# agordon/fastx_toolkit

Measured on AMD Instinct MI355X. Metric: Mreads/s (150 bp) quality-trim+filter, higher is better.
Workload: dtype u8

## Files before the change

fastx_toolkit_amd/csrc/fxg_device.h:

```cpp
#pragma once
#include <hip/hip_runtime.h>
#include <stdint.h>
#include <cstdio>
#include <cstring>

#include "../../include/fxg.h"

typedef unsigned int       u32;
typedef unsigned long long u64;
typedef unsigned int u32x4 __attribute__((ext_vector_type(4)));

#define FXG_HD __host__ __device__ __forceinline__
#define FXG_PLAN_FAIL(...) do { snprintf(err, cap, __VA_ARGS__); return FXG_E_INVALID; } while (0)
static inline int fxg_text_check_len(unsigned long long text_len, char *err, size_t cap) { if (text_len > 0xFFFFFFF0ull) FXG_PLAN_FAIL("text block too large (%llu bytes)", text_len); return FXG_OK; }
static inline bool fxg_text_lpr_ok(int lpr) { return lpr == 4 || lpr == 2; }

#if defined(FXG_ABLATION) || defined(FXG_DBG_BITS)
#define FXG_DBG(a, bit) ((a).debug & (bit))
#else
#define FXG_DBG(a, bit) 0u
#endif

#define FXG_BLOCK 256
#define FXG_WAVES (FXG_BLOCK / 64)
// ... 64 lines not shown
    u32  nf_keep_n;
    u32  rev_dw;
    u64 *extra;
    const uint8_t  *clip_src;
    u64  clip_total;
    u32  clip_stride;
    const uint16_t *wlen;
    float *clip_ck;
    u32  clip_ck_rows;
    u32  clip_ptab_rows;
    u32  clip_ptab_stride;
    u32  clip_ptab_cols;
    u32  clip_ptab_dia1;
    char adapter[100];
    uint8_t clip_ptab_row[256];
};

__device__ __forceinline__ u32 fxg_lane() { return threadIdx.x & 63u; }

FXG_HD u32 fxg_ge_flags(u32 w, u32 K) { return (((w & 0x7f7f7f7fu) + K) | w) & 0x80808080u; }

FXG_HD u32 fxg_pack4(u32 f)
{
    u32 t = f >> 7;
    t |= t >> 7;
    t |= t >> 14;
    return t & 0xFu;
}

FXG_HD u32 fxg_mask16(u32x4 v, u32 K)
// ... 549 lines not shown
```

fastx_toolkit_amd/csrc/fxg_engine.hip:

```cpp
#include "fxg_host.h"
#include "fxg_text.h"
#include "fxg_history.h"
#include "fxg_stats.h"
#include "fxg_fallback.h"
#include "fxg_barcode.h"
#include "fxg_reflow.h"

extern "C" int fxg_abi_version(void) { return FXG_ABI_VERSION; }

extern "C" int fxg_ctx_create(int device_id, fxg_ctx **out)
{
    if (!out) return FXG_E_INVALID;
    *out = nullptr;
    int ndev = 0;
    if (hipGetDeviceCount(&ndev) != hipSuccess || ndev <= 0 || device_id < 0 || device_id >= ndev) return FXG_E_HIP;
    fxg_ctx *c = (fxg_ctx *)calloc(1, sizeof(fxg_ctx));
    if (!c) return FXG_E_NOMEM;
    c->device = device_id;
    hipDeviceProp_t prop;
    if (hipSetDevice(device_id) != hipSuccess || hipGetDeviceProperties(&prop, device_id) != hipSuccess ||
        hipStreamCreateWithFlags(&c->own_stream, hipStreamNonBlocking) != hipSuccess) { fxg_ctx_destroy(c); return FXG_E_HIP; }
    c->cus = prop.multiProcessorCount;
    c->stream = c->own_stream;
    { const char *e = getenv("FXG_BLOCKS_PER_CU"); c->env_blocks_per_cu = (e && atoi(e) > 0 && atoi(e) <= 16) ? atoi(e) : 0; }
    { const char *e = getenv("FXG_WORKERS"); c->env_workers = (e && atoi(e) > 0) ? atoi(e) : 0; }
    { const char *e = getenv("FXG_NSCAN"); c->env_nscan = (e && atoi(e) > 0 && atoi(e) <= 64) ? atoi(e) : 0; }
    { const char *e = getenv("FXG_TEST_SCAN_TIMEOUT"); c->test_force_timeout = (e && atoi(e) > 0) ? 1 : 0; }
    { const char *e = getenv("FXG_TICKET_GROUPS"); c->env_ticket_groups = (e && atoi(e) > 0 && atoi(e) <= FXG_TICKET_GROUPS) ? atoi(e) : 0; }
    if (hipEventCreate(&c->ev0) != hipSuccess || hipEventCreate(&c->ev1) != hipSuccess ||
        hipMalloc((void **)&c->errflag, (FXG_CTRL_WORDS + FXG_TICKET_GROUPS * FXG_TICKET_STRIDE) * sizeof(u32)) != hipSuccess ||
        hipMalloc((void **)&c->counters_scratch, FXG_NCOUNTERS * sizeof(u64)) != hipSuccess) { fxg_ctx_destroy(c); return FXG_E_HIP; }
    *out = c;
    return FXG_OK;
}

extern "C" void fxg_ctx_destroy(fxg_ctx *c)
{
    if (!c) return;
    (void)hipSetDevice(c->device);
    if (c->stream) (void)hipStreamSynchronize(c->stream);
    (void)hipFree(c->status); (void)hipFree(c->errflag); (void)hipFree(c->counters_scratch);
// ... 152 lines not shown
    return fxg_launch_plan(c, pl, (u64 *)out->counters);
}

static int fxg_launch_clip(fxg_ctx *c, FxgPlan &pl, u64 *ctr)
{
    int rc;
#define FXG_CLIP_TRY_UNIT(K) if ((rc = FXG_CLIP_UNIT_FN(K)(c, pl, ctr)) != FXG_CLIP_NOT_MINE) return rc;
    FXG_CLIP_FOR_UNITS(FXG_CLIP_TRY_UNIT)
#undef FXG_CLIP_TRY_UNIT
    return fxg_fail(c, FXG_E_INVALID, "no clip instance %d", pl.amax);
}

static int fxg_launch_plan(fxg_ctx *c, FxgPlan &pl, u64 *ctr)
{
    if (pl.rows_nw) {
        if (pl.rows_h == 2) {
            if (pl.rows_nw == 26) return fxg_launch_tiles(c, fxg_kernel_rows<26, 2>, "fxg_kernel_rows<26,2> qtrim+qfilter", pl.ka, pl.lds, ctr, 64u, true);
            return fxg_launch_tiles(c, fxg_kernel_rows<38, 2>, "fxg_kernel_rows<38,2> qtrim+qfilter", pl.ka, pl.lds, ctr, 64u, true);
        }
        switch (pl.rows_nw) {
        case 10: return fxg_launch_tiles(c, fxg_kernel_rows_multi<10, 4>, "fxg_kernel_rows_multi<10,4> qtrim+qfilter", pl.ka, pl.lds, ctr, 64u, true);
        case 14: return fxg_launch_tiles(c, fxg_kernel_rows_multi<14, 3>, "fxg_kernel_rows_multi<14,3> qtrim+qfilter", pl.ka, pl.lds, ctr, 64u, true);
        case 20: return fxg_launch_tiles(c, fxg_kernel_rows_multi<20, 2>, "fxg_kernel_rows_multi<20,2> qtrim+qfilter", pl.ka, pl.lds, ctr, 64u, true);
        case 26: return fxg_launch_tiles(c, fxg_kernel_rows<26>, "fxg_kernel_rows<26> qtrim+qfilter", pl.ka, pl.lds, ctr, 64u, true);
        default: return fxg_launch_tiles(c, fxg_kernel_rows<38>, "fxg_kernel_rows<38> qtrim+qfilter", pl.ka, pl.lds, ctr, 64u, true);
        }
    }
    if (pl.group_a) {
        if (pl.amax == 0) return fxg_launch_tiles(c, fxg_kernel_tiles<0, 0>, "fxg_kernel_tiles<0,0> qtrim+qfilter", pl.ka, pl.lds, ctr);
        return fxg_launch_clip(c, pl, ctr);
    }
    if (pl.mask) return fxg_launch_tiles(c, fxg_kernel_tiles<0, 3>, "fxg_kernel_tiles<0,3> mask", pl.ka, pl.lds, ctr);
    if (pl.artifacts) return fxg_launch_tiles(c, fxg_kernel_tiles<0, 4>, "fxg_kernel_tiles<0,4> base census", pl.ka, pl.lds, ctr);
    if (pl.rev && pl.ka.rev_dw) return fxg_launch_tiles(c, fxg_kernel_tiles<0, 5>, "fxg_kernel_tiles<0,5> revcomp[+ftrim], dword-aligned windows", pl.ka, pl.lds, ctr);
    if (pl.rev) return fxg_launch_tiles(c, fxg_kernel_tiles<0, 2>, "fxg_kernel_tiles<0,2> revcomp[+ftrim]", pl.ka, pl.lds, ctr);
    return fxg_launch_tiles(c, fxg_kernel_tiles<0, 1>, "fxg_kernel_tiles<0,1> ftrim", pl.ka, pl.lds, ctr);
}

extern "C" int fxg_run_quality_stats(fxg_ctx *c, const fxg_batch *in, uint64_t *d_hist, uint32_t hist_cols)
{
    if (!c) return FXG_E_INVALID;
// ... 530 lines not shown
```

fastx_toolkit_amd/csrc/fxg_host.h:

```cpp
#pragma once
#include <hip/hip_runtime.h>

#include <dlfcn.h>
#include <fcntl.h>
#include <cerrno>
#include <cstdarg>
#include <cstdio>
#include <cstdlib>
#include <cstring>
#include <unistd.h>

#include "fxg_plan.h"
#include "fxg_rows.h"

struct FxgTextState;

struct fxg_ctx {
    int device;
    int cus;
    hipStream_t own_stream;
    hipStream_t stream;
    hipEvent_t ev0, ev1;
#define FXG_KEV_RING 64
    hipEvent_t kev0[FXG_KEV_RING], kev1[FXG_KEV_RING];
    int profiling;
    u64 kev_count;
    int kev_ready;
    u64 *status;
    size_t status_cap;
    u32 epoch;
    void *attr_kernel[8];
    u32 attr_lds[8];
    int attr_per_cu[8];
    int attr_next;
    void *lds_kernel[32];
    u32 lds_max[32];
    int env_blocks_per_cu, env_ticket_groups;
    int env_workers, env_nscan;
    u32 *errflag;
    u64 *counters_scratch;
    u64 *text_ws;
    size_t text_ws_cap;
    FxgTextState *text_state;
    int hist_on;
    u32 hist_wcap;
    int hist_cur;
    uint8_t *hist_buf[2];
    u32 *hist_w;
    uint8_t *hist_ws;
    size_t hist_ws_cap;
    float *clip_ck;
    size_t clip_ck_cap;
    u32 *stats_ws;
// ... 68 lines not shown
        FXG_HIP(c, hipFuncSetAttribute((const void *)kernel, hipFuncAttributeMaxDynamicSharedMemorySize, (int)lds));
        if (k >= 0) { c->lds_kernel[k] = (void *)kernel; c->lds_max[k] = lds; }
    }
    FXG_HIP(c, hipOccupancyMaxActiveBlocksPerMultiprocessor(per_cu, kernel, (int)block, lds));
    if (*per_cu < 1) return fxg_fail(c, FXG_E_INVALID, "%s does not fit on a CU (lds=%u)", kname, lds);
    int slot = -1;
    for (int i = 0; i < 8; ++i) if (!c->attr_kernel[i]) { slot = i; break; }
    if (slot < 0) { slot = c->attr_next; c->attr_next = (c->attr_next + 1) % 8; }
    c->attr_kernel[slot] = (void *)kernel; c->attr_lds[slot] = lds; c->attr_per_cu[slot] = *per_cu;
    return FXG_OK;
}

#define FXG_STATUS_WORDS(cap) (3 * (size_t)(cap) + 2 * ((size_t)(cap) / 256 + 2))

template <typename K>
static int fxg_launch_tiles(fxg_ctx *c, K kernel, const char *kname, FxgKArgs &ka, u32 lds, u64 *counters, u32 block = FXG_TBLOCK, bool rows_kernel = false, u64 ck_per_wg = 0)
{
    FXG_HIP(c, hipSetDevice(c->device));
    int per_cu = 0;
    FXG_TRY(fxg_kernel_fit(c, kernel, kname, lds, &per_cu, block));
    const int most = block == 64u ? 16 : 8;
    int use = per_cu > most ? most : per_cu;
    if (c->env_blocks_per_cu > 0) use = c->env_blocks_per_cu;
    u64 workers = (u64)c->cus * (u64)use;
    if (c->env_workers > 0 && workers > (u64)c->env_workers) workers = (u64)c->env_workers;
    if (workers > ka.ntiles) workers = ka.ntiles;
    if (workers < 1) workers = 1;
    ka.nscan = !ka.compact ? 0u : (rows_kernel && workers >= 64u * FXG_ROWS_NSCAN ? (u32)FXG_ROWS_NSCAN : 1u);
    if (ka.compact && rows_kernel && c->env_nscan > 0) ka.nscan = (u32)c->env_nscan;
    const u64 grid = workers + ka.nscan;

    if (ka.compact) {
        bool fresh = false;
        const size_t cap = (size_t)ka.ntiles + (size_t)ka.ntiles / 4 + 1024;
        FXG_TRY(fxg_ws_grow(c, c->status, c->status_cap, ka.ntiles, cap, &fresh, FXG_STATUS_WORDS(cap) * sizeof(u64)));
        c->epoch = c->epoch >= 255u ? 1u : c->epoch + 1u;
        if (fresh || c->epoch == 1u) FXG_HIP(c, hipMemsetAsync(c->status, 0, FXG_STATUS_WORDS(c->status_cap) * sizeof(u64), c->stream));
        ka.agg = c->status;
        ka.pfx = c->status + c->status_cap;
        ka.bbase = c->status + 3 * c->status_cap;
        ka.tag = c->epoch;
    }
    ka.clip_ck = nullptr;
    if (ck_per_wg) {
        const size_t need = (size_t)grid * (size_t)ck_per_wg;
        FXG_TRY(fxg_ws_grow(c, c->clip_ck, c->clip_ck_cap, need, need));
        ka.clip_ck = c->clip_ck;
    }
#if defined(FXG_ABLATION) || defined(FXG_DBG_BITS)
    { const char *dbg = getenv("FXG_DEBUG"); ka.debug = dbg ? (u32)atoi(dbg) : 0u; }
#endif
    ka.errflag = c->errflag;
    ka.ticket = c->errflag + FXG_CTRL_WORDS;
    ka.extra = (u64 *)(c->errflag + 2);
    ka.role = c->errflag + 8;
    ka.tally = (u64 *)(c->errflag + 32);
    { u32 g = c->env_ticket_groups > 0 ? (u32)c->env_ticket_groups : FXG_TICKET_GROUPS; ka.ticket_groups = grid >= (u64)(ka.nscan + 1u) * g ? g : 1u; }
    FXG_HIP(c, hipMemsetAsync(c->errflag, 0, (FXG_CTRL_WORDS + FXG_TICKET_GROUPS * FXG_TICKET_STRIDE) * sizeof(u32), c->stream));
    c->fb.valid = 0;
    if (ka.compact) {
        c->fb.ka = ka; c->fb.counters = counters; c->fb.valid = 1;
        if (c->test_force_timeout) {
            static const u32 up = FXG_DEV_ERR_SCAN_TIMEOUT;
            FXG_HIP(c, hipMemcpyAsync(c->errflag, &up, sizeof up, hipMemcpyHostToDevice, c->stream));
        }
    }

    if (c->profiling) FXG_HIP(c, hipEventRecord(c->kev0[c->kev_count % FXG_KEV_RING], c->stream));
    FXG_LAUNCH(c, kernel, (u32)grid, block, lds, ka);
    if (c->profiling) { FXG_HIP(c, hipEventRecord(c->kev1[c->kev_count % FXG_KEV_RING], c->stream)); c->kev_count++; }
    FXG_TRY(fxg_enqueue_finish_counters(c, ka, counters));
    snprintf(c->last_kernel, sizeof c->last_kernel, "%s", kname);
// ... 4 lines not shown
```

fastx_toolkit_amd/csrc/fxg_plan.h:

```cpp
#pragma once
#include <cstdio>
#include <cstdlib>
#include <cstring>

#include "fxg_clip_instances.h"
#include "fxg_kernels.h"
#include "fxg_rows.h"

static_assert(fxg_clip_bucket(1) != 0 && fxg_clip_bucket(FXG_MAX_ADAPTER) != 0, "every adapter length the plan accepts needs a packed clip instance");

struct FxgPlan {
    FxgKArgs ka;
    bool group_a;
    bool clip, use_q, rev;
    bool mask, artifacts;
    int  amax;
    u32  lds;
    int  rows_nw;
    int  rows_h;
    int  rows_r;
    u32  block;
    u64  ck_per_wg;
};

static inline int fxg_clampi(long long v, int lo, int hi) { return v < lo ? lo : (v > hi ? hi : (int)v); }

static inline u32 fxg_pick_tile(u32 stride, bool clip, u32 block = FXG_TBLOCK)
{
    const u64 budget = clip ? 60ull * 1024 : 20ull * 1024;
    u32 T = block;
    const char *env = getenv("FXG_TILE");
    if (env && atoi(env) >= 1 && atoi(env) <= (int)block && (atoi(env) & (atoi(env) - 1)) == 0) return (u32)atoi(env);
    while (T > 1 && (u64)T * stride > budget) T >>= 1;
    return T;
}
// ... 82 lines not shown
        }
    }
    pl->rows_nw = 0; pl->rows_h = 1; pl->rows_r = 1;
    {
        const int want = getenv("FXG_ROWS") ? atoi(getenv("FXG_ROWS")) : 1;
        const u32 top = want >= 2 ? 304u : 208u;
        if (ga && !pl->clip && ka.compact && in->stride >= 80u && in->stride <= top && want != 0) {
            pl->rows_h = in->stride <= 152u ? 1 : 2;
            pl->rows_nw = in->stride <= 104u * (u32)pl->rows_h ? 26 : 38;
        } else if (ga && !pl->clip && ka.compact && in->stride >= 28u && in->stride < 80u && want != 0) {
            if (in->stride <= 40u) { pl->rows_nw = 10; pl->rows_r = 4; }
            else if (in->stride <= 56u) { pl->rows_nw = 14; pl->rows_r = 3; }
            else { pl->rows_nw = 20; pl->rows_r = 2; }
        }
    }
    pl->block = pl->rows_nw ? 64u : (ga && pl->amax < 0 && pl->amax >= -16) ? (u32)FXG_CLIP_TBLOCK : (u32)FXG_TBLOCK;
    ka.clip_global = 0u;
    u32 T = pl->rows_nw ? 64u * (u32)pl->rows_r / (u32)pl->rows_h : fxg_pick_tile(pl->clip ? ka.clip_stride : in->stride, pl->clip, pl->block);
    if (pl->clip && pl->amax < 0 && (pl->amax >= -16 || pl->ck_per_wg != 0) && clip_stride == 0u && (ka.clip_stride & 3u) == 0u && ((uintptr_t)ka.clip_src & 3u) == 0u) {
        ka.tile_reads = T; ka.depth = 2u;
        const bool cramped = T < pl->block || (156u * 1024u) / fxg_plan_lds(pl) < 3u;
        const char *e = getenv("FXG_CLIP_GLOBAL");
        ka.clip_global = (e ? atoi(e) != 0 : cramped) ? 1u : 0u;
        if (ka.clip_global) T = pl->block;
    }
    const u64 ntiles = (in->n + T - 1) / T;
    if (ntiles > 0x7FFFFFFFull || in->n > 0xFFFFFFFFull) FXG_PLAN_FAIL("batch too large (%llu reads): split it", (unsigned long long)in->n);
    ka.tile_reads = T; ka.ntiles = (u32)ntiles;
    ka.rev_dw = 0u;
    if ((st & FXG_STAGE_REVCOMP) && !in->len && (T & 3u) == 0u) {
// ... 44 lines not shown
```

fastx_toolkit_amd/csrc/fxg_rows.h:

```cpp
#pragma once
#include "fxg_kernels.h"

#define FXG_ROWS_T 64u
#ifndef FXG_ROWS_LB
#define FXG_ROWS_LB 3
#endif
#ifndef FXG_ROWS_SCAN_K
#define FXG_ROWS_SCAN_K 8
#endif
#ifndef FXG_ROWS_LD_AUX
#define FXG_ROWS_LD_AUX 2
#endif
#ifndef FXG_ROWS_NSCAN
#define FXG_ROWS_NSCAN 8
#endif
#ifndef FXG_ROWS_SPARSE_BASES
#define FXG_ROWS_SPARSE_BASES 1
#endif
#define FXG_ROWS_SPARSE_MULTI (FXG_ROWS_SPARSE_BASES >= 2)

__host__ __device__ inline u32 fxg_rows_lds(u32 stride, u32 lanes_per_read = 1u, u32 reads_per_lane = 1u) { return fxg_r16(FXG_ROWS_T * reads_per_lane / lanes_per_read * stride) + 176u; }

template <int NW>
FXG_HD void fxg_rows_bits(const u32 (&row)[NW], u32 K, u32 (&M)[(NW * 4 + 31) / 32])
{
#pragma unroll
    for (int p = 0; p < (NW + 1) / 2; ++p) {
        const u32 f0 = fxg_ge_flags(row[2 * p], K), f1 = 2 * p + 1 < NW ? fxg_ge_flags(row[2 * p + 1], K) : 0u;
#ifndef FXG_HOST_EMULATION
        const u32 b = __builtin_amdgcn_udot4(f1, 0x80402010u, __builtin_amdgcn_udot4(f0, 0x08040201u, 0u, false), false);
#else
        u32 b = 0;
        for (int i = 0; i < 4; ++i) b += ((f0 >> (8 * i)) & 0xFFu) * (1u << i) + ((f1 >> (8 * i)) & 0xFFu) * (16u << i);
#endif
        if ((p & 3) == 0) M[p >> 2] = b >> 7;
        else M[p >> 2] |= b << (8 * (p & 3) - 7);
// ... 101 lines not shown
    u32 m = 0;
#pragma unroll
    for (int K = 0; K < NC; ++K) {
        const u32 b0 = 1024u * (u32)K + 16u * lane;
        m |= fxg_rows_needed<H, R>(b0, b0 + 15u, stride, magic, perm) ? 1u << K : 0u;
    }
    if (tbytes & 3u) {
        const u32 x = (tbytes & ~3u) + lane;
        m |= fxg_rows_needed<H, R>(x, x, stride, magic, perm) ? FXG_ROWS_TAIL_BIT : 0u;
    }
    return m;
}

#ifndef FXG_HOST_EMULATION
typedef __attribute__((address_space(3))) unsigned char fxg_lds_u8;
#define FXG_WAVE_SYNC() do { __builtin_amdgcn_fence(__ATOMIC_RELEASE, "wavefront"); asm volatile("s_waitcnt lgkmcnt(0)" ::: "memory"); __builtin_amdgcn_wave_barrier(); __builtin_amdgcn_fence(__ATOMIC_ACQUIRE, "wavefront"); } while (0)

template <int K, int NC, bool SPARSE>
__device__ __forceinline__ void fxg_rows_fetch_from(__amdgpu_buffer_rsrc_t rs, fxg_lds_u8 *sbuf, u32 lane, u32 nck, u32 room, u32 need)
{
    typedef __attribute__((address_space(3))) void lptr_t;
    if constexpr (K < NC) {
        if constexpr (SPARSE) {
            if ((u32)K < nck && ((need >> K) & 1u) && ((u32)(K + 1) * 1024u <= room || (u32)K * 1024u + (lane << 4) < room)) __builtin_amdgcn_raw_ptr_buffer_load_lds(rs, (lptr_t *)(sbuf + (K >> 2) * 4096), 16, (int)(lane << 4) + (K >> 2) * 4096, 0, (K & 3) * 1024, FXG_ROWS_LD_AUX);
        } else {
            if ((u32)K < nck && ((u32)(K + 1) * 1024u <= room || (u32)K * 1024u + (lane << 4) < room)) __builtin_amdgcn_raw_ptr_buffer_load_lds(rs, (lptr_t *)(sbuf + (K >> 2) * 4096), 16, (int)(lane << 4) + (K >> 2) * 4096, 0, (K & 3) * 1024, FXG_ROWS_LD_AUX);
        }
        fxg_rows_fetch_from<K + 1, NC, SPARSE>(rs, sbuf, lane, nck, room, need);
    }
}
// ... 101 lines not shown
        fxg_st16_stream(g0 + ((u64)i << 4), o);
    }
    const bool whole = end > first;
    const u32 hb = whole ? (sh ? 16u - sh : 0u) : totb;
    const u32 ts = whole ? (end << 4) - sh : totb;
    if (lane < hb) out[base + lane] = obuf[lane];
    if (ts + lane < totb) out[base + ts + lane] = obuf[ts + lane];
}

#ifdef FXG_ABLATION
#define FXG_PHASE(i) do { const u64 now_ = __builtin_amdgcn_s_memrealtime(); ph[i] += now_ - pt; pt = now_; } while (0)
#else
#define FXG_PHASE(i) do { } while (0)
#endif

template <int NW, int H = 1>
__global__ __launch_bounds__(64, FXG_ROWS_LB) void fxg_kernel_rows(const FxgKArgs a)
{
    constexpr u32 TR = FXG_ROWS_T / (u32)H, HB = 4u * (u32)NW;
    extern __shared__ __attribute__((aligned(16))) unsigned char smem[];
    fxg_lds_u8 *lsm = (fxg_lds_u8 *)smem;
    u32 lane = threadIdx.x;
    const u32 stride = a.stride;
#if FXG_ROWS_SPARSE_BASES
    const u32 magic = fxg_rows_magic(stride);
#endif
    u32 role = 0;
    if (lane == 0) role = atomicAdd(a.role, 1u);
    role = (u32)__builtin_amdgcn_readfirstlane((int)role);
    if (role < a.nscan) { if (a.nscan == 1u) fxg_scanner_k<FXG_ROWS_SCAN_K>(a); else fxg_scanner_multi<FXG_ROWS_SCAN_K>(a, role); return; }
    const u32 G = a.ticket_groups, grp = blockIdx.x % G;
    u32 *my_ticket = a.ticket + grp * FXG_TICKET_STRIDE;
    u32 tk = 0;
    if (lane == 0) tk = atomicAdd(my_ticket, 1u);
    u32 cur = (u32)__builtin_amdgcn_readfirstlane((int)tk) * G + grp;
    u64 t_in = 0, t_kept = 0, t_bases = 0, t_qtrim = 0, t_qfilter = 0;
#ifdef FXG_ABLATION
    u64 ph[8] = {0, 0, 0, 0, 0, 0, 0, 0}, pt = __builtin_amdgcn_s_memrealtime();
#endif
    u32 qp[NW];
    u32 p_info = 0, p_exc = 0, p_totb = 0, pend = FXG_NO_TILE;
    for (;;) {
        asm volatile("" : "+v"(lane));
        const bool havec = cur < a.ntiles, havep = pend != FXG_NO_TILE;
        u32 q[NW];
        u32 c_info = 0, c_exc = 0, c_totb = 0;
        if (havec) {
            const u32 r0 = cur * TR;
            const u64 left = a.n - (u64)r0;
            const u32 nreads = left < (u64)TR ? (u32)left : TR;
            const u64 tb = (u64)r0 * stride;
            const u32 tbytes = nreads * stride;
            const u32 rd = lane / (u32)H, hf = lane % (u32)H;
            fxg_rows_fetch<NW>(a.qual, tb, tbytes, lsm, lane);
            fxg_rows_landed();
            FXG_PHASE(0);
            fxg_rows_read<NW>(smem, rd * stride + hf * HB, q);
            FXG_WAVE_SYNC();
            u32 keep = 0, olen = 0, word = 0;
// ... 28 lines not shown
            const u32 tot = (u32)__builtin_amdgcn_readlane((int)inc, 63);
            const u32 totc = tot >> 16;
            c_totb = tot & 0xFFFFu;
            c_exc = (inc - mine) >> 16;
            c_info = ((keep && (H == 1 || hf == 0u || olen)) ? 1u << 31 : 0u) | (olen << 16) | ((inc - mine) & 0xFFFFu);
            if (lane == 0) fxg_publish_total(a, cur, totc, c_totb);
            t_in += nreads; t_kept += totc; t_bases += c_totb;
            FXG_PHASE(1);
        }
        u64 bc[2] = {0, 0};
        if (havep) {
            if (!FXG_DBG(a, 2u)) fxg_wait_prefix_wave(a, pend, bc); else { bc[0] = (u64)pend * TR; bc[1] = bc[0] * stride; }
            FXG_PHASE(2);
        }
        u32 nxt = 0;
        if (havec && lane == 0) nxt = atomicAdd(my_ticket, 1u);
        if (havep) {
            const u32 r0 = pend * TR;
            const u64 left = a.n - (u64)r0;
            const u32 nreads = left < (u64)TR ? (u32)left : TR;
            const u64 tb = (u64)r0 * stride;
            const u32 tbytes = nreads * stride;
            const u32 rd = lane / (u32)H, hf = lane % (u32)H;
            const bool placed = bc[0] != ~0ull;
            const u32 keep = placed ? p_info >> 31 : 0u, olen = (p_info >> 16) & 0x7FFFu, exb = p_info & 0xFFFFu;
            const bool fast = __ballot(keep && olen < 4u) == 0ull;
            if (keep && !FXG_DBG(a, 64u)) fxg_rows_pack<NW>(smem, exb, qp, olen, fast);
            FXG_WAVE_SYNC();
            FXG_PHASE(6);
            if (placed && !FXG_DBG(a, 1u)) fxg_rows_flush(a.out_qual, bc[1], p_totb, smem, lane);
            if constexpr (H == 1) { if (keep) fxg_write_kept_meta(a, bc[0] + p_exc, olen, r0 + lane, bc[1] + exb); }
// ... 15 lines not shown
                need = fxg_rows_base_need<NW, H, 1>(kw, lane, stride, magic, tbytes);
#endif
                fxg_rows_fetch<NW, FXG_ROWS_SPARSE_BASES != 0>(a.bases, tb, tbytes, lsm, lane, need);
                fxg_rows_landed();
                FXG_PHASE(4);
                fxg_rows_read<NW>(smem, rd * stride + hf * HB, b);
                FXG_WAVE_SYNC();
                if (keep && !FXG_DBG(a, 64u)) fxg_rows_pack<NW>(smem, exb, b, olen, fast);
                FXG_WAVE_SYNC();
                FXG_PHASE(7);
                if (placed && !FXG_DBG(a, 1u)) fxg_rows_flush(a.out_bases, bc[1], p_totb, smem, lane);
                FXG_WAVE_SYNC();
            }
            FXG_PHASE(5);
        }
        if (!havec) break;
#pragma unroll
        for (int k = 0; k < NW; ++k) qp[k] = q[k];
        p_info = c_info; p_exc = c_exc; p_totb = c_totb; pend = cur;
        cur = (u32)__builtin_amdgcn_readfirstlane((int)nxt) * G + grp;
    }
#ifdef FXG_ABLATION
    if (lane == 0) for (int i = 0; i < 8; ++i) atomicAdd(reinterpret_cast<u64 *>(a.errflag + 10) + i, ph[i]);
#endif
    if (lane == 0) {
        if (t_in) atomicAdd(&a.tally[0], t_in);
        if (t_kept) atomicAdd(&a.tally[1], t_kept);
        if (t_bases) atomicAdd(&a.tally[2], t_bases);
        if (t_qtrim) atomicAdd(&a.tally[4 + FXG_R_QTRIM], t_qtrim);
        if (t_qfilter) atomicAdd(&a.tally[4 + FXG_R_QFILTER], t_qfilter);
    }
}
template <int NW, int R>
__global__ __launch_bounds__(64, FXG_ROWS_LB) void fxg_kernel_rows_multi(const FxgKArgs a)
{
    constexpr u32 TR = FXG_ROWS_T * (u32)R;
    extern __shared__ __attribute__((aligned(16))) unsigned char smem[];
    fxg_lds_u8 *lsm = (fxg_lds_u8 *)smem;
    u32 lane = threadIdx.x;
    const u32 stride = a.stride;
#if FXG_ROWS_SPARSE_MULTI
    const u32 magic = fxg_rows_magic(stride);
#endif
    u32 role = 0;
    if (lane == 0) role = atomicAdd(a.role, 1u);
    role = (u32)__builtin_amdgcn_readfirstlane((int)role);
    if (role < a.nscan) { if (a.nscan == 1u) fxg_scanner_k<FXG_ROWS_SCAN_K>(a); else fxg_scanner_multi<FXG_ROWS_SCAN_K>(a, role); return; }
    const u32 G = a.ticket_groups, grp = blockIdx.x % G;
    u32 *my_ticket = a.ticket + grp * FXG_TICKET_STRIDE;
    u32 tk = 0;
    if (lane == 0) tk = atomicAdd(my_ticket, 1u);
    u32 cur = (u32)__builtin_amdgcn_readfirstlane((int)tk) * G + grp;
    u64 t_in = 0, t_kept = 0, t_bases = 0, t_qtrim = 0, t_qfilter = 0;
    u32 qp[R][NW];
    u32 p_info[R], p_exc[R], p_totb = 0, pend = FXG_NO_TILE;
#pragma unroll
    for (int j = 0; j < R; ++j) { p_info[j] = 0u; p_exc[j] = 0u; }
    for (;;) {
        asm volatile("" : "+v"(lane));
        const bool havec = cur < a.ntiles, havep = pend != FXG_NO_TILE;
        u32 q[R][NW];
        u32 c_info[R], c_exc[R], c_totb = 0;
#pragma unroll
        for (int j = 0; j < R; ++j) { c_info[j] = 0u; c_exc[j] = 0u; }
        if (havec) {
            const u32 r0 = cur * TR;
            const u64 left = a.n - (u64)r0;
            const u32 nreads = left < (u64)TR ? (u32)left : TR;
            const u64 tb = (u64)r0 * stride;
            const u32 tbytes = nreads * stride;
            fxg_rows_fetch<NW * R>(a.qual, tb, tbytes, lsm, lane);
            fxg_rows_landed();
#pragma unroll
            for (int j = 0; j < R; ++j) fxg_rows_read<NW>(smem, ((u32)j * FXG_ROWS_T + lane) * stride, q[j]);
            FXG_WAVE_SYNC();
// ... 9 lines not shown
                const u32 mine = keep ? ((1u << 16) | olen) : 0u;
                const u32 inc = fxg_wave_scan_dpp(mine);
                const u32 ex = inc - mine + base;
                base += (u32)__builtin_amdgcn_readlane((int)inc, 63);
                c_exc[j] = ex >> 16;
                c_info[j] = (keep ? 1u << 31 : 0u) | (olen << 16) | (ex & 0xFFFFu);
            }
            const u32 totc = base >> 16;
            c_totb = base & 0xFFFFu;
            if (lane == 0) fxg_publish_total(a, cur, totc, c_totb);
            t_in += nreads; t_kept += totc; t_bases += c_totb;
        }
        u64 bc[2] = {0, 0};
        if (havep) fxg_wait_prefix_wave(a, pend, bc);
        u32 nxt = 0;
        if (havec && lane == 0) nxt = atomicAdd(my_ticket, 1u);
        if (havep) {
            const u32 r0 = pend * TR;
            const u64 left = a.n - (u64)r0;
            const u32 nreads = left < (u64)TR ? (u32)left : TR;
            const u64 tb = (u64)r0 * stride;
            const u32 tbytes = nreads * stride;
            const bool placed = bc[0] != ~0ull;
            u64 shortm = 0;
#pragma unroll
            for (int j = 0; j < R; ++j) shortm |= __ballot(placed && (p_info[j] >> 31) && ((p_info[j] >> 16) & 0x7FFFu) < 4u);
            const bool fast = shortm == 0ull;
#pragma unroll
            for (int j = 0; j < R; ++j) {
                const u32 keep = placed ? p_info[j] >> 31 : 0u, olen = (p_info[j] >> 16) & 0x7FFFu, exb = p_info[j] & 0xFFFFu;
                if (keep) fxg_rows_pack<NW>(smem, exb, qp[j], olen, fast);
// ... 18 lines not shown
                fxg_rows_fetch<NW * R, FXG_ROWS_SPARSE_MULTI>(a.bases, tb, tbytes, lsm, lane, need);
                fxg_rows_landed();
#pragma unroll
                for (int j = 0; j < R; ++j) fxg_rows_read<NW>(smem, ((u32)j * FXG_ROWS_T + lane) * stride, b[j]);
                FXG_WAVE_SYNC();
#pragma unroll
                for (int j = 0; j < R; ++j) {
                    const u32 keep = placed ? p_info[j] >> 31 : 0u, olen = (p_info[j] >> 16) & 0x7FFFu, exb = p_info[j] & 0xFFFFu;
                    if (keep) fxg_rows_pack<NW>(smem, exb, b[j], olen, fast);
                }
                FXG_WAVE_SYNC();
                if (placed) fxg_rows_flush(a.out_bases, bc[1], p_totb, smem, lane);
                FXG_WAVE_SYNC();
            }
        }
        if (!havec) break;
#pragma unroll
        for (int j = 0; j < R; ++j) {
#pragma unroll
            for (int k = 0; k < NW; ++k) qp[j][k] = q[j][k];
            p_info[j] = c_info[j]; p_exc[j] = c_exc[j];
        }
        p_totb = c_totb; pend = cur;
        cur = (u32)__builtin_amdgcn_readfirstlane((int)nxt) * G + grp;
    }
    if (lane == 0) {
        if (t_in) atomicAdd(&a.tally[0], t_in);
        if (t_kept) atomicAdd(&a.tally[1], t_kept);
        if (t_bases) atomicAdd(&a.tally[2], t_bases);
        if (t_qtrim) atomicAdd(&a.tally[4 + FXG_R_QTRIM], t_qtrim);
        if (t_qfilter) atomicAdd(&a.tally[4 + FXG_R_QFILTER], t_qfilter);
    }
}
#endif
```

Measured before the change: 13120.

## Add multi-wave workgroups and chunked ticket-to-tile mapping for rows kernels

Generalises the rows kernels so several independent waves can share one workgroup, drawing tiles through a shared LDS ticket, with separate LDS slices per wave. It also adds a chunked ticket-to-tile mapping so consecutive tickets within a ticket group cover runs of adjacent tiles. By default the workgroup width stays 1, but the 38-word family uses a chunk of 8. The aim is to improve tile locality and scheduling, at the cost of a more complex work distribution and extra barriers when grouping is enabled.

```diff
diff --git a/fastx_toolkit_amd/csrc/fxg_device.h b/fastx_toolkit_amd/csrc/fxg_device.h
--- a/fastx_toolkit_amd/csrc/fxg_device.h
+++ b/fastx_toolkit_amd/csrc/fxg_device.h
@@ -102,6 +102,8 @@
     u32  clip_ptab_dia1;
     char adapter[100];
     uint8_t clip_ptab_row[256];
+    u32  rows_chunk;
+    u32  rows_lds;
 };
 
 __device__ __forceinline__ u32 fxg_lane() { return threadIdx.x & 63u; }
diff --git a/fastx_toolkit_amd/csrc/fxg_engine.hip b/fastx_toolkit_amd/csrc/fxg_engine.hip
--- a/fastx_toolkit_amd/csrc/fxg_engine.hip
+++ b/fastx_toolkit_amd/csrc/fxg_engine.hip
@@ -25,6 +25,8 @@
     { const char *e = getenv("FXG_BLOCKS_PER_CU"); c->env_blocks_per_cu = (e && atoi(e) > 0 && atoi(e) <= 16) ? atoi(e) : 0; }
     { const char *e = getenv("FXG_WORKERS"); c->env_workers = (e && atoi(e) > 0) ? atoi(e) : 0; }
     { const char *e = getenv("FXG_NSCAN"); c->env_nscan = (e && atoi(e) > 0 && atoi(e) <= 64) ? atoi(e) : 0; }
+    { const char *e = getenv("FXG_ROWS_WG"); c->env_rows_wg = (e && atoi(e) > 0 && atoi(e) <= FXG_ROWS_WG_MAX) ? atoi(e) : 0; }
+    { const char *e = getenv("FXG_ROWS_CHUNK"); c->env_rows_chunk = (e && atoi(e) > 0 && atoi(e) <= 4096) ? atoi(e) : 0; }
     { const char *e = getenv("FXG_TEST_SCAN_TIMEOUT"); c->test_force_timeout = (e && atoi(e) > 0) ? 1 : 0; }
     { const char *e = getenv("FXG_TICKET_GROUPS"); c->env_ticket_groups = (e && atoi(e) > 0 && atoi(e) <= FXG_TICKET_GROUPS) ? atoi(e) : 0; }
     if (hipEventCreate(&c->ev0) != hipSuccess || hipEventCreate(&c->ev1) != hipSuccess ||
@@ -207,17 +209,19 @@
 static int fxg_launch_plan(fxg_ctx *c, FxgPlan &pl, u64 *ctr)
 {
     if (pl.rows_nw) {
+#define FXG_ROWS_LAUNCH(KERNEL, A, B, NAME) return fxg_launch_tiles(c, KERNEL<A, B>, NAME, pl.ka, pl.lds, ctr, 64u, true, 0, pl.rows_wg, pl.rows_chunk, KERNEL##_wg<A, B>)
         if (pl.rows_h == 2) {
-            if (pl.rows_nw == 26) return fxg_launch_tiles(c, fxg_kernel_rows<26, 2>, "fxg_kernel_rows<26,2> qtrim+qfilter", pl.ka, pl.lds, ctr, 64u, true);
-            return fxg_launch_tiles(c, fxg_kernel_rows<38, 2>, "fxg_kernel_rows<38,2> qtrim+qfilter", pl.ka, pl.lds, ctr, 64u, true);
+            if (pl.rows_nw == 26) FXG_ROWS_LAUNCH(fxg_kernel_rows, 26, 2, "fxg_kernel_rows<26,2> qtrim+qfilter");
+            FXG_ROWS_LAUNCH(fxg_kernel_rows, 38, 2, "fxg_kernel_rows<38,2> qtrim+qfilter");
         }
         switch (pl.rows_nw) {
-        case 10: return fxg_launch_tiles(c, fxg_kernel_rows_multi<10, 4>, "fxg_kernel_rows_multi<10,4> qtrim+qfilter", pl.ka, pl.lds, ctr, 64u, true);
-        case 14: return fxg_launch_tiles(c, fxg_kernel_rows_multi<14, 3>, "fxg_kernel_rows_multi<14,3> qtrim+qfilter", pl.ka, pl.lds, ctr, 64u, true);
-        case 20: return fxg_launch_tiles(c, fxg_kernel_rows_multi<20, 2>, "fxg_kernel_rows_multi<20,2> qtrim+qfilter", pl.ka, pl.lds, ctr, 64u, true);
-        case 26: return fxg_launch_tiles(c, fxg_kernel_rows<26>, "fxg_kernel_rows<26> qtrim+qfilter", pl.ka, pl.lds, ctr, 64u, true);
-        default: return fxg_launch_tiles(c, fxg_kernel_rows<38>, "fxg_kernel_rows<38> qtrim+qfilter", pl.ka, pl.lds, ctr, 64u, true);
+        case 10: FXG_ROWS_LAUNCH(fxg_kernel_rows_multi, 10, 4, "fxg_kernel_rows_multi<10,4> qtrim+qfilter");
+        case 14: FXG_ROWS_LAUNCH(fxg_kernel_rows_multi, 14, 3, "fxg_kernel_rows_multi<14,3> qtrim+qfilter");
+        case 20: FXG_ROWS_LAUNCH(fxg_kernel_rows_multi, 20, 2, "fxg_kernel_rows_multi<20,2> qtrim+qfilter");
+        case 26: FXG_ROWS_LAUNCH(fxg_kernel_rows, 26, 1, "fxg_kernel_rows<26> qtrim+qfilter");
+        default: FXG_ROWS_LAUNCH(fxg_kernel_rows, 38, 1, "fxg_kernel_rows<38> qtrim+qfilter");
         }
+#undef FXG_ROWS_LAUNCH
     }
     if (pl.group_a) {
         if (pl.amax == 0) return fxg_launch_tiles(c, fxg_kernel_tiles<0, 0>, "fxg_kernel_tiles<0,0> qtrim+qfilter", pl.ka, pl.lds, ctr);
diff --git a/fastx_toolkit_amd/csrc/fxg_host.h b/fastx_toolkit_amd/csrc/fxg_host.h
--- a/fastx_toolkit_amd/csrc/fxg_host.h
+++ b/fastx_toolkit_amd/csrc/fxg_host.h
@@ -37,6 +37,7 @@
     u32 lds_max[32];
     int env_blocks_per_cu, env_ticket_groups;
     int env_workers, env_nscan;
+    int env_rows_wg, env_rows_chunk;
     u32 *errflag;
     u64 *counters_scratch;
     u64 *text_ws;
@@ -135,7 +136,8 @@
 #define FXG_STATUS_WORDS(cap) (3 * (size_t)(cap) + 2 * ((size_t)(cap) / 256 + 2))
 
 template <typename K>
-static int fxg_launch_tiles(fxg_ctx *c, K kernel, const char *kname, FxgKArgs &ka, u32 lds, u64 *counters, u32 block = FXG_TBLOCK, bool rows_kernel = false, u64 ck_per_wg = 0)
+static int fxg_launch_tiles(fxg_ctx *c, K kernel, const char *kname, FxgKArgs &ka, u32 lds, u64 *counters, u32 block = FXG_TBLOCK, bool rows_kernel = false, u64 ck_per_wg = 0,
+                            u32 rows_wg = 1u, u32 rows_chunk = 1u, K kernel_wg = nullptr)
 {
     FXG_HIP(c, hipSetDevice(c->device));
     int per_cu = 0;
@@ -143,13 +145,31 @@
     const int most = block == 64u ? 16 : 8;
     int use = per_cu > most ? most : per_cu;
     if (c->env_blocks_per_cu > 0) use = c->env_blocks_per_cu;
+    u32 W = 1u, C = 1u;
+    if (rows_kernel) {
+        const bool capped = (c->env_workers > 0 || c->env_blocks_per_cu > 0) && c->env_rows_wg == 0;
+        W = c->env_rows_wg > 0 ? (u32)c->env_rows_wg : capped ? 1u : rows_wg;
+        C = c->env_rows_chunk > 0 ? (u32)c->env_rows_chunk : capped ? 1u : rows_chunk;
+        if (!kernel_wg || W > (u32)FXG_ROWS_WG_MAX || (u32)use % W != 0u) W = 1u;
+        if (W > 1u) {
+            int wg_per_cu = 0;
+            if (fxg_kernel_fit(c, kernel_wg, kname, lds * W, &wg_per_cu, block * W) != FXG_OK || wg_per_cu < use / (int)W) W = 1u;
+        }
+        if (W > 1u) kernel = kernel_wg;
+        ka.rows_chunk = C; ka.rows_lds = lds;
+    }
     u64 workers = (u64)c->cus * (u64)use;
     if (c->env_workers > 0 && workers > (u64)c->env_workers) workers = (u64)c->env_workers;
-    if (workers > ka.ntiles) workers = ka.ntiles;
-    if (workers < 1) workers = 1;
+    u64 wgs = workers / W;
+    const u64 wg_tiles = ((u64)ka.ntiles + W - 1u) / W;
+    if (wgs > wg_tiles) wgs = wg_tiles;
+    if (wgs < 1) wgs = 1;
+    workers = wgs * W;
     ka.nscan = !ka.compact ? 0u : (rows_kernel && workers >= 64u * FXG_ROWS_NSCAN ? (u32)FXG_ROWS_NSCAN : 1u);
     if (ka.compact && rows_kernel && c->env_nscan > 0) ka.nscan = (u32)c->env_nscan;
-    const u64 grid = workers + ka.nscan;
+    const u32 scan_wgs = (ka.nscan + W - 1u) / W;
+    const u64 grid = wgs + scan_wgs;
+    block *= W; lds *= W;
 
     if (ka.compact) {
         bool fresh = false;
@@ -176,7 +196,7 @@
     ka.extra = (u64 *)(c->errflag + 2);
     ka.role = c->errflag + 8;
     ka.tally = (u64 *)(c->errflag + 32);
-    { u32 g = c->env_ticket_groups > 0 ? (u32)c->env_ticket_groups : FXG_TICKET_GROUPS; ka.ticket_groups = grid >= (u64)(ka.nscan + 1u) * g ? g : 1u; }
+    { u32 g = c->env_ticket_groups > 0 ? (u32)c->env_ticket_groups : FXG_TICKET_GROUPS; ka.ticket_groups = grid >= (u64)(scan_wgs + 1u) * g ? g : 1u; }
     FXG_HIP(c, hipMemsetAsync(c->errflag, 0, (FXG_CTRL_WORDS + FXG_TICKET_GROUPS * FXG_TICKET_STRIDE) * sizeof(u32), c->stream));
     c->fb.valid = 0;
     if (ka.compact) {
diff --git a/fastx_toolkit_amd/csrc/fxg_plan.h b/fastx_toolkit_amd/csrc/fxg_plan.h
--- a/fastx_toolkit_amd/csrc/fxg_plan.h
+++ b/fastx_toolkit_amd/csrc/fxg_plan.h
@@ -19,6 +19,7 @@
     int  rows_nw;
     int  rows_h;
     int  rows_r;
+    u32  rows_wg, rows_chunk;
     u32  block;
     u64  ck_per_wg;
 };
@@ -131,6 +132,11 @@
             else { pl->rows_nw = 20; pl->rows_r = 2; }
         }
     }
+    {
+        const bool fam38 = pl->rows_nw == 38 && pl->rows_h == 1;
+        pl->rows_wg = fam38 ? (u32)FXG_ROWS_WG_38 : (u32)FXG_ROWS_WG_OTHER;
+        pl->rows_chunk = fam38 ? (u32)FXG_ROWS_CHUNK_38 : (u32)FXG_ROWS_CHUNK_OTHER;
+    }
     pl->block = pl->rows_nw ? 64u : (ga && pl->amax < 0 && pl->amax >= -16) ? (u32)FXG_CLIP_TBLOCK : (u32)FXG_TBLOCK;
     ka.clip_global = 0u;
     u32 T = pl->rows_nw ? 64u * (u32)pl->rows_r / (u32)pl->rows_h : fxg_pick_tile(pl->clip ? ka.clip_stride : in->stride, pl->clip, pl->block);
diff --git a/fastx_toolkit_amd/csrc/fxg_rows.h b/fastx_toolkit_amd/csrc/fxg_rows.h
--- a/fastx_toolkit_amd/csrc/fxg_rows.h
+++ b/fastx_toolkit_amd/csrc/fxg_rows.h
@@ -14,12 +14,27 @@
 #ifndef FXG_ROWS_NSCAN
 #define FXG_ROWS_NSCAN 8
 #endif
+#define FXG_ROWS_WG_MAX 12
+#ifndef FXG_ROWS_WG_38
+#define FXG_ROWS_WG_38 1
+#endif
+#ifndef FXG_ROWS_CHUNK_38
+#define FXG_ROWS_CHUNK_38 8
+#endif
+#define FXG_ROWS_WG_OTHER 1
+#define FXG_ROWS_CHUNK_OTHER 1
 #ifndef FXG_ROWS_SPARSE_BASES
 #define FXG_ROWS_SPARSE_BASES 1
 #endif
 #define FXG_ROWS_SPARSE_MULTI (FXG_ROWS_SPARSE_BASES >= 2)
 
 __host__ __device__ inline u32 fxg_rows_lds(u32 stride, u32 lanes_per_read = 1u, u32 reads_per_lane = 1u) { return fxg_r16(FXG_ROWS_T * reads_per_lane / lanes_per_read * stride) + 176u; }
+
+FXG_HD u32 fxg_rows_tile_of(u32 ticket, u32 group, u32 groups, u32 chunk, u32 wg_waves, u32 wave)
+{
+    const u32 run = chunk > 1u ? ((ticket / chunk) * groups + group) * chunk + ticket % chunk : ticket * groups + group;
+    return wg_waves > 1u ? run * wg_waves + wave : run;
+}
 
 template <int NW>
 FXG_HD void fxg_rows_bits(const u32 (&row)[NW], u32 K, u32 (&M)[(NW * 4 + 31) / 32])
@@ -151,6 +166,7 @@
 
 #ifndef FXG_HOST_EMULATION
 typedef __attribute__((address_space(3))) unsigned char fxg_lds_u8;
+typedef volatile __attribute__((address_space(3))) u32 fxg_lds_vu32;
 #define FXG_WAVE_SYNC() do { __builtin_amdgcn_fence(__ATOMIC_RELEASE, "wavefront"); asm volatile("s_waitcnt lgkmcnt(0)" ::: "memory"); __builtin_amdgcn_wave_barrier(); __builtin_amdgcn_fence(__ATOMIC_ACQUIRE, "wavefront"); } while (0)
 
 template <int K, int NC, bool SPARSE>
@@ -282,26 +298,44 @@
 #define FXG_PHASE(i) do { } while (0)
 #endif
 
-template <int NW, int H = 1>
-__global__ __launch_bounds__(64, FXG_ROWS_LB) void fxg_kernel_rows(const FxgKArgs a)
+__device__ __forceinline__ bool fxg_rows_scanner_role(const FxgKArgs &a, u32 W, u32 wave, u32 lane, fxg_lds_vu32 *wgw)
+{
+    u32 role = 0;
+    if (W == 1u) {
+        if (lane == 0) role = atomicAdd(a.role, 1u);
+        role = (u32)__builtin_amdgcn_readfirstlane((int)role);
+    } else {
+        if (wave == 0u && lane == 0) wgw[2] = atomicAdd(a.role, 1u);
+        __syncthreads();
+        role = (u32)__builtin_amdgcn_readfirstlane((int)wgw[2]) * W + wave;
+    }
+    if (role < a.nscan) { if (a.nscan == 1u) fxg_scanner_k<FXG_ROWS_SCAN_K>(a); else fxg_scanner_multi<FXG_ROWS_SCAN_K>(a, role); return true; }
+    return role - wave < a.nscan;
+}
+
+template <int NW, int H, bool GRP>
+__device__ __forceinline__ void fxg_rows_body(const FxgKArgs a)
 {
     constexpr u32 TR = FXG_ROWS_T / (u32)H, HB = 4u * (u32)NW;
-    extern __shared__ __attribute__((aligned(16))) unsigned char smem[];
+    extern __shared__ __attribute__((aligned(16))) unsigned char smem_wg[];
+    __shared__ u32 wgw_[4];
+    fxg_lds_vu32 *wgw = (fxg_lds_vu32 *)wgw_;
+    const u32 W = GRP ? blockDim.x >> 6 : 1u, wave = GRP ? (u32)__builtin_amdgcn_readfirstlane((int)(threadIdx.x >> 6)) : 0u;
+    unsigned char *smem = smem_wg + wave * a.rows_lds;
     fxg_lds_u8 *lsm = (fxg_lds_u8 *)smem;
-    u32 lane = threadIdx.x;
+    u32 lane = threadIdx.x & 63u;
     const u32 stride = a.stride;
 #if FXG_ROWS_SPARSE_BASES
     const u32 magic = fxg_rows_magic(stride);
 #endif
-    u32 role = 0;
-    if (lane == 0) role = atomicAdd(a.role, 1u);
-    role = (u32)__builtin_amdgcn_readfirstlane((int)role);
-    if (role < a.nscan) { if (a.nscan == 1u) fxg_scanner_k<FXG_ROWS_SCAN_K>(a); else fxg_scanner_multi<FXG_ROWS_SCAN_K>(a, role); return; }
-    const u32 G = a.ticket_groups, grp = blockIdx.x % G;
+    if (fxg_rows_scanner_role(a, W, wave, lane, wgw)) return;
+    const u32 G = a.ticket_groups, grp = blockIdx.x % G, C = a.rows_chunk;
     u32 *my_ticket = a.ticket + grp * FXG_TICKET_STRIDE;
-    u32 tk = 0;
-    if (lane == 0) tk = atomicAdd(my_ticket, 1u);
-    u32 cur = (u32)__builtin_amdgcn_readfirstlane((int)tk) * G + grp;
+    u32 tk = 0, rnd = 0, drawn = 0;
+    if (wave == 0u && lane == 0) drawn = atomicAdd(my_ticket, 1u);
+    if (W == 1u) tk = (u32)__builtin_amdgcn_readfirstlane((int)drawn);
+    else if (wave == 0u && lane == 0) wgw[0] = drawn;
+    u32 cur = 0;
     u64 t_in = 0, t_kept = 0, t_bases = 0, t_qtrim = 0, t_qfilter = 0;
 #ifdef FXG_ABLATION
     u64 ph[8] = {0, 0, 0, 0, 0, 0, 0, 0}, pt = __builtin_amdgcn_s_memrealtime();
@@ -310,7 +344,12 @@
     u32 p_info = 0, p_exc = 0, p_totb = 0, pend = FXG_NO_TILE;
     for (;;) {
         asm volatile("" : "+v"(lane));
-        const bool havec = cur < a.ntiles, havep = pend != FXG_NO_TILE;
+        if (W > 1u) {
+            __syncthreads();
+            tk = (u32)__builtin_amdgcn_readfirstlane((int)wgw[rnd & 1u]);
+        }
+        cur = fxg_rows_tile_of(tk, grp, G, C, W, wave);
+        const bool havew = cur - wave < a.ntiles, havec = cur < a.ntiles, havep = pend != FXG_NO_TILE;
         u32 q[NW];
         u32 c_info = 0, c_exc = 0, c_totb = 0;
         if (havec) {
@@ -369,7 +408,7 @@
             FXG_PHASE(2);
         }
         u32 nxt = 0;
-        if (havec && lane == 0) nxt = atomicAdd(my_ticket, 1u);
+        if (havew && wave == 0u && lane == 0) nxt = atomicAdd(my_ticket, 1u);
         if (havep) {
             const u32 r0 = pend * TR;
             const u64 left = a.n - (u64)r0;
@@ -415,11 +454,12 @@
             }
             FXG_PHASE(5);
         }
-        if (!havec) break;
+        if (!havew) break;
 #pragma unroll
         for (int k = 0; k < NW; ++k) qp[k] = q[k];
-        p_info = c_info; p_exc = c_exc; p_totb = c_totb; pend = cur;
-        cur = (u32)__builtin_amdgcn_readfirstlane((int)nxt) * G + grp;
+        p_info = c_info; p_exc = c_exc; p_totb = c_totb; pend = havec ? cur : FXG_NO_TILE;
+        if (W == 1u) tk = (u32)__builtin_amdgcn_readfirstlane((int)nxt);
+        else { ++rnd; if (wave == 0u && lane == 0) wgw[rnd & 1u] = nxt; }
     }
 #ifdef FXG_ABLATION
     if (lane == 0) for (int i = 0; i < 8; ++i) atomicAdd(reinterpret_cast<u64 *>(a.errflag + 10) + i, ph[i]);
@@ -432,26 +472,33 @@
         if (t_qfilter) atomicAdd(&a.tally[4 + FXG_R_QFILTER], t_qfilter);
     }
 }
-template <int NW, int R>
-__global__ __launch_bounds__(64, FXG_ROWS_LB) void fxg_kernel_rows_multi(const FxgKArgs a)
+template <int NW, int H = 1>
+__global__ __launch_bounds__(64, FXG_ROWS_LB) void fxg_kernel_rows(const FxgKArgs a) { fxg_rows_body<NW, H, false>(a); }
+template <int NW, int H = 1>
+__global__ __launch_bounds__(64 * FXG_ROWS_WG_MAX, FXG_ROWS_LB) void fxg_kernel_rows_wg(const FxgKArgs a) { fxg_rows_body<NW, H, true>(a); }
+template <int NW, int R, bool GRP>
+__device__ __forceinline__ void fxg_rows_multi_body(const FxgKArgs a)
 {
     constexpr u32 TR = FXG_ROWS_T * (u32)R;
-    extern __shared__ __attribute__((aligned(16))) unsigned char smem[];
+    extern __shared__ __attribute__((aligned(16))) unsigned char smem_wg[];
+    __shared__ u32 wgw_[4];
+    fxg_lds_vu32 *wgw = (fxg_lds_vu32 *)wgw_;
+    const u32 W = GRP ? blockDim.x >> 6 : 1u, wave = GRP ? (u32)__builtin_amdgcn_readfirstlane((int)(threadIdx.x >> 6)) : 0u;
+    unsigned char *smem = smem_wg + wave * a.rows_lds;
     fxg_lds_u8 *lsm = (fxg_lds_u8 *)smem;
-    u32 lane = threadIdx.x;
+    u32 lane = threadIdx.x & 63u;
     const u32 stride = a.stride;
 #if FXG_ROWS_SPARSE_MULTI
     const u32 magic = fxg_rows_magic(stride);
 #endif
-    u32 role = 0;
-    if (lane == 0) role = atomicAdd(a.role, 1u);
-    role = (u32)__builtin_amdgcn_readfirstlane((int)role);
-    if (role < a.nscan) { if (a.nscan == 1u) fxg_scanner_k<FXG_ROWS_SCAN_K>(a); else fxg_scanner_multi<FXG_ROWS_SCAN_K>(a, role); return; }
-    const u32 G = a.ticket_groups, grp = blockIdx.x % G;
+    if (fxg_rows_scanner_role(a, W, wave, lane, wgw)) return;
+    const u32 G = a.ticket_groups, grp = blockIdx.x % G, C = a.rows_chunk;
     u32 *my_ticket = a.ticket + grp * FXG_TICKET_STRIDE;
-    u32 tk = 0;
-    if (lane == 0) tk = atomicAdd(my_ticket, 1u);
-    u32 cur = (u32)__builtin_amdgcn_readfirstlane((int)tk) * G + grp;
+    u32 tk = 0, rnd = 0, drawn = 0;
+    if (wave == 0u && lane == 0) drawn = atomicAdd(my_ticket, 1u);
+    if (W == 1u) tk = (u32)__builtin_amdgcn_readfirstlane((int)drawn);
+    else if (wave == 0u && lane == 0) wgw[0] = drawn;
+    u32 cur = 0;
     u64 t_in = 0, t_kept = 0, t_bases = 0, t_qtrim = 0, t_qfilter = 0;
     u32 qp[R][NW];
     u32 p_info[R], p_exc[R], p_totb = 0, pend = FXG_NO_TILE;
@@ -459,7 +506,12 @@
     for (int j = 0; j < R; ++j) { p_info[j] = 0u; p_exc[j] = 0u; }
     for (;;) {
         asm volatile("" : "+v"(lane));
-        const bool havec = cur < a.ntiles, havep = pend != FXG_NO_TILE;
+        if (W > 1u) {
+            __syncthreads();
+            tk = (u32)__builtin_amdgcn_readfirstlane((int)wgw[rnd & 1u]);
+        }
+        cur = fxg_rows_tile_of(tk, grp, G, C, W, wave);
+        const bool havew = cur - wave < a.ntiles, havec = cur < a.ntiles, havep = pend != FXG_NO_TILE;
         u32 q[R][NW];
         u32 c_info[R], c_exc[R], c_totb = 0;
 #pragma unroll
@@ -499,7 +551,7 @@
         u64 bc[2] = {0, 0};
         if (havep) fxg_wait_prefix_wave(a, pend, bc);
         u32 nxt = 0;
-        if (havec && lane == 0) nxt = atomicAdd(my_ticket, 1u);
+        if (havew && wave == 0u && lane == 0) nxt = atomicAdd(my_ticket, 1u);
         if (havep) {
             const u32 r0 = pend * TR;
             const u64 left = a.n - (u64)r0;
@@ -548,15 +600,16 @@
                 FXG_WAVE_SYNC();
             }
         }
-        if (!havec) break;
+        if (!havew) break;
 #pragma unroll
         for (int j = 0; j < R; ++j) {
 #pragma unroll
             for (int k = 0; k < NW; ++k) qp[j][k] = q[j][k];
             p_info[j] = c_info[j]; p_exc[j] = c_exc[j];
         }
-        p_totb = c_totb; pend = cur;
-        cur = (u32)__builtin_amdgcn_readfirstlane((int)nxt) * G + grp;
+        p_totb = c_totb; pend = havec ? cur : FXG_NO_TILE;
+        if (W == 1u) tk = (u32)__builtin_amdgcn_readfirstlane((int)nxt);
+        else { ++rnd; if (wave == 0u && lane == 0) wgw[rnd & 1u] = nxt; }
     }
     if (lane == 0) {
         if (t_in) atomicAdd(&a.tally[0], t_in);
@@ -566,4 +619,8 @@
         if (t_qfilter) atomicAdd(&a.tally[4 + FXG_R_QFILTER], t_qfilter);
     }
 }
-#endif
+template <int NW, int R>
+__global__ __launch_bounds__(64, FXG_ROWS_LB) void fxg_kernel_rows_multi(const FxgKArgs a) { fxg_rows_multi_body<NW, R, false>(a); }
+template <int NW, int R>
+__global__ __launch_bounds__(64 * FXG_ROWS_WG_MAX, FXG_ROWS_LB) void fxg_kernel_rows_multi_wg(const FxgKArgs a) { fxg_rows_multi_body<NW, R, true>(a); }
+#endif
```

Result: faster. 13270, median of 6 (+1.1%).
